# andrewrosemberg/DiffOpt.jl

Hardware: AMD Instinct MI355X
Metric: KKT sensitivity solves/sec (fwd+rev) on batched QPs (higher is better)
Workload: dtype f64; 1 GPU; config 2: dense QP batch, fwd+rev sensitivities; problems_per_gpu=1024, n=200, m_ineq=300, p_eq=0, parallelism=batch-sharded x1

## Files before the change

diffopt.jl_amd/csrc/dopt_internal.h:

```cpp
#pragma once
#include <hip/hip_runtime.h>

#include <cstdint>
#include <functional>
#include <string>
#include <vector>

#include "../../include/diffopt_mi355x.h"

#define DOPT_CHECK_HIP(expr)                                                   \
  do {                                                                         \
    hipError_t _e = (expr);                                                    \
    if (_e != hipSuccess) {                                                    \
      throw dopt::Error(-2, std::string(#expr) + ": " + hipGetErrorString(_e)); \
    }                                                                          \
  } while (0)

namespace dopt {

struct Error {
  int code;
  std::string msg;
  Error(int c, std::string m) : code(c), msg(std::move(m)) {}
};
// ... 5 lines not shown
    if (nbytes <= bytes && p) return;
    if (p) (void)hipFree(p);
    p = nullptr;
    bytes = 0;
    if (nbytes == 0) return;
    DOPT_CHECK_HIP(hipMalloc(&p, nbytes));
    bytes = nbytes;
  }
  void release() {
    if (p) (void)hipFree(p);
    p = nullptr;
    bytes = 0;
  }
  template <class T>
  T* as() const { return static_cast<T*>(p); }
};

enum QPLu { LU_NONE = 0, LU_NOPIV = 1, LU_PIVOT = 2, LU_REJECT = 3, LU_GENERIC = 4, LU_SMALL = 5 };
constexpr int LU_SEL_NOPIV = 1 << LU_NOPIV;
constexpr int LU_SEL_PIVOT = 1 << LU_PIVOT;
constexpr int LU_SEL_ALL = LU_SEL_NOPIV | LU_SEL_PIVOT;
struct QPMeta {
  int32_t nk;
  int32_t nsys;
  int32_t iterative;
  int32_t info;
  int32_t lu;
  int32_t gk_ok;
  int32_t sym;
  int32_t spec_miss;
};

constexpr int ASM_WPP = 16;
constexpr int SM_MAX = 128;
constexpr int SM_BATCH = 8;
constexpr int DENSE_QP_MAX = 8192;
constexpr int BLOCKED_MAX = 4096;
constexpr int PIVOT_MAX = 1536;

enum QPRoute { ROUTE_LSQR = 0, ROUTE_BLOCKED = 2, ROUTE_GENERIC = 3 };
__host__ __device__ inline int qp_route(int iterative, int nsys) {
  if (iterative) return ROUTE_LSQR;
  if (nsys <= BLOCKED_MAX) return ROUTE_BLOCKED;
  return ROUTE_GENERIC;
}

constexpr double NOPIV_LMAX = 10.0;
constexpr double NOPIV_GROWTH = 1e8;

__device__ __forceinline__ double add_mul_rn(double x, double y, double z) {
#pragma clang fp contract(off)
  return x + y * z;
}
__device__ __forceinline__ double sub_rn(double x, double y) {
#pragma clang fp contract(off)
  return x - y;
}

struct PScale {
  const double* kl;
  int n, nk;
  __device__ double operator()(int r) const {
    if (!kl) return 1.0;
    const bool in = r >= n && r < n + nk;
    const double v = kl[in ? r - n : 0];
    return in ? v : 1.0;
// ... 327 lines not shown
```

diffopt.jl_amd/csrc/qp.hip:

```cpp
#include "device_prims.h"
#include "lsqr_core.h"
#include "qp_assemble.h"

namespace dopt {

constexpr int TPB = 256;
constexpr int OUT_LCAP = 4096;
constexpr int NB = 32;

__global__ __launch_bounds__(TPB) void qp_lu_generic_kernel(
    double* __restrict__ K, int32_t* __restrict__ ipiv, QPMeta* __restrict__ meta,
    int nmax, int ld, const int32_t* __restrict__ plist) {
  __shared__ double redv[4];
  __shared__ int redi[4];
  const int b = plist[blockIdx.x], t = threadIdx.x;
  const int lane = t & 63, wv = t >> 6;
  const int N = meta[b].nsys;
  double* Kb = K + (size_t)b * nmax * ld;
  int32_t* piv = ipiv + (size_t)b * nmax;
  int info = 0;
  for (int j = 0; j < N; ++j) {
    double best = -1.0;
    int bi = 0x7fffffff;
    for (int r = j + t; r < N; r += TPB) {
// ... 194 lines not shown
__global__ __launch_bounds__(TPB) void qp_lsqr_kernel(
    const double* __restrict__ K, const QPMeta* __restrict__ meta, int nmax,
    int ld, int trans, const double* __restrict__ rhs, double* __restrict__ xout,
    double* __restrict__ work) {
  __shared__ double red[4];
  const int b = blockIdx.x, t = threadIdx.x;
  if (!meta[b].iterative) return;
  const int N = meta[b].nsys;
  const double* Kb = K + (size_t)b * nmax * ld;
  double* x = work + (size_t)b * 5 * nmax;
  double* u = x + N;
  double* v = u + N;
  double* w = v + N;
  double* tmp = w + N;
  const DenseKKT op{Kb, ld, N, trans};
  LsqrScalars st;
  lsqr_solve<TPB, block_sum>(st, op, rhs + (size_t)b * nmax, 0.0, N, x, u, v, w, tmp, N, red);
  __syncthreads();
  for (int i = t; i < N; i += TPB) xout[(size_t)b * nmax + i] = x[i];
}

__global__ __launch_bounds__(TPB) void qp_rev_rhs_kernel(
    const double* __restrict__ dl_dz, const QPMeta* __restrict__ meta, int n,
    int nmax, double* __restrict__ rhs, double* __restrict__ rhs2) {
  const int b = blockIdx.x, t = threadIdx.x;
  const int N = meta[b].nsys;
  for (int i = t; i < N; i += TPB) {
    const double v = (i < n) ? dl_dz[(size_t)b * n + i] : 0.0;
    rhs[(size_t)b * nmax + i] = v;
    if (rhs2) rhs2[(size_t)b * nmax + i] = v;
  }
}

__global__ __launch_bounds__(TPB) void qp_fwd_rhs_kernel(
    const double* __restrict__ dQ, const double* __restrict__ dq,
    const double* __restrict__ dG, const double* __restrict__ dh,
    const double* __restrict__ dA, const double* __restrict__ db,
    const double* __restrict__ z, const double* __restrict__ lam,
    const double* __restrict__ nu, const int32_t* __restrict__ rpos,
    const QPMeta* __restrict__ meta, int n, int m, int p, int nmax, int zcap,
    double* __restrict__ full, double* __restrict__ rhs, double* __restrict__ rhs2) {
  extern __shared__ __attribute__((aligned(16))) double smem[];
  const int b = blockIdx.x, t = threadIdx.x, lane = t & 63, wv = t >> 6;
  const double* zg = z + (size_t)b * n;
  const double* lb = lam + (size_t)b * m;
  const double* nb = nu + (size_t)b * p;
  const bool staged = n <= zcap;
  if (staged)
    for (int i = t; i < n; i += TPB) smem[i] = zg[i];
  __syncthreads();
  const double* zs = staged ? smem : zg;
  double* r = full + (size_t)b * nmax;
  for (int i = t; i < n; i += TPB) {
    double acc = 0.0;
    if (dQ) {
      const double* Qb = dQ + (size_t)b * n * n;
      for (int j = 0; j < n; ++j) acc = fma(Qb[i + (size_t)j * n], zs[j], acc);
    }
    if (dq) acc += dq[(size_t)b * n + i];
    r[i] = acc;
  }
  __syncthreads();
  if (dG && m > 0) {
    const double* Gb = dG + (size_t)b * m * n;
    for (int i = wv; i < n; i += 4) {
      double acc = 0.0;
      for (int l = lane; l < m; l += 64) acc = fma(Gb[l + (size_t)i * m], lb[l], acc);
      acc = wave_sum(acc);
      if (lane == 0) r[i] += acc;
    }
  }
  __syncthreads();
  if (dA && p > 0) {
    const double* Ab = dA + (size_t)b * p * n;
    for (int i = wv; i < n; i += 4) {
      double acc = 0.0;
      for (int l = lane; l < p; l += 64) acc = fma(Ab[l + (size_t)i * p], nb[l], acc);
      acc = wave_sum(acc);
      if (lane == 0) r[i] += acc;
    }
  }
  for (int l = t; l < m; l += TPB) {
    double gz = 0.0;
    if (dG) {
      const double* Gb = dG + (size_t)b * m * n;
      for (int j = 0; j < n; ++j) gz = fma(Gb[l + (size_t)j * m], zs[j], gz);
    }
    const double hh = dh ? dh[(size_t)b * m + l] : 0.0;
    r[n + l] = lb[l] * gz - lb[l] * hh;
  }
  for (int e = t; e < p; e += TPB) {
    double az = 0.0;
    if (dA) {
      const double* Ab = dA + (size_t)b * p * n;
      for (int j = 0; j < n; ++j) az = fma(Ab[e + (size_t)j * p], zs[j], az);
    }
    r[n + m + e] = az - (db ? db[(size_t)b * p + e] : 0.0);
  }
  __syncthreads();
  const int nk = meta[b].nk;
  double* rb = rhs + (size_t)b * nmax;
  double* rb2 = rhs2 ? rhs2 + (size_t)b * nmax : nullptr;
  for (int i = t; i < n; i += TPB) {
    rb[i] = r[i];
    if (rb2) rb2[i] = r[i];
  }
  for (int l = t; l < m; l += TPB) {
    const int kk = rpos[(size_t)b * m + l];
    if (kk >= 0) {
      rb[n + kk] = r[n + l];
      if (rb2) rb2[n + kk] = r[n + l];
    }
  }
  for (int e = t; e < p; e += TPB) {
    rb[n + nk + e] = r[n + m + e];
    if (rb2) rb2[n + nk + e] = r[n + m + e];
  }
}

#ifndef DOPT_QP_NT
#define DOPT_QP_NT 0
#endif
__global__ __launch_bounds__(TPB) void qp_output_kernel(
    const double* __restrict__ x0, const double* __restrict__ G,
    const double* __restrict__ s, const int32_t* __restrict__ rpos,
    const QPMeta* __restrict__ meta, const double* __restrict__ full, int n,
    int m, int p, int nmax, int zcap, int trans0, double* __restrict__ out0, const double* __restrict__ x1,
    double* __restrict__ out1, int B) {
  extern __shared__ __attribute__((aligned(16))) double smem[];
  __shared__ int nel;
  const bool second = x1 && (int)blockIdx.x >= B;
  const int b = second ? (int)blockIdx.x - B : (int)blockIdx.x, t = threadIdx.x;
  const double* __restrict__ x = second ? x1 : x0;
  double* __restrict__ out = second ? out1 : out0;
  const int trans = second ? 1 : trans0;
  const int nk = meta[b].nk;
  const double* xb = x + (size_t)b * nmax;
  double* ob = out + (size_t)b * (n + m + p);
  const bool staged = n <= zcap;
  const double* xz = staged ? smem : xb;
  int* el = reinterpret_cast<int*>(smem + (staged ? n : 0));
  const bool listed = !trans && m <= OUT_LCAP;
  if (t == 0) nel = 0;
  for (int i = t; i < n; i += TPB) {
    if (staged) smem[i] = xb[i];
    ob[i] = -xb[i];
  }
  for (int e = t; e < p; e += TPB) ob[n + m + e] = -xb[n + nk + e];
  __syncthreads();
  const double* Gb = G + (size_t)b * m * n;
  const double* sb = s + (size_t)b * m;
  auto elim_row = [&](int l) {
    double acc = 0.0;
    int j = 0;
    for (; j + 8 <= n; j += 8) {
      double gv[8];
#pragma unroll
      for (int u = 0; u < 8; ++u)
        gv[u] = DOPT_QP_NT ? __builtin_nontemporal_load(&Gb[l + (size_t)(j + u) * m]) : Gb[l + (size_t)(j + u) * m];
#pragma unroll
      for (int u = 0; u < 8; ++u) acc = fma(gv[u], xz[j + u], acc);
    }
    for (; j < n; ++j) acc = fma(Gb[l + (size_t)j * m], xz[j], acc);
    ob[n + l] = -((0.0 - acc) / sb[l]);
  };
  for (int l = t; l < m; l += TPB) {
    const int kk = rpos[(size_t)b * m + l];
    if (kk >= 0) {
      ob[n + l] = -xb[n + kk];
    } else if (!trans) {
      if (listed) el[atomicAdd(&nel, 1)] = l;
      else elim_row(l);
    } else {
      ob[n + l] = -(full[(size_t)b * nmax + n + l] / sb[l]);
    }
  }
  if (!listed) return;
  __syncthreads();
  for (int e = t; e < nel; e += TPB) elim_row(el[e]);
}

constexpr int OKC = 16;
__global__ __launch_bounds__(TPB) void qp_output_k_kernel(
    const double* __restrict__ x, const double* __restrict__ G, const double* __restrict__ s,
    const int32_t* __restrict__ rpos, const QPMeta* __restrict__ meta, const double* __restrict__ full,
    int B, int k, int n, int m, int p, int nmax, int trans, double* __restrict__ out) {
  extern __shared__ __attribute__((aligned(16))) double smem[];
  const int b = blockIdx.x, t = threadIdx.x;
  const int j0 = blockIdx.y * OKC, kc = min(OKC, k - j0);
  const int nk = meta[b].nk;
  const size_t L = (size_t)n + m + p;
  const bool staged = !trans && n * OKC * 8 <= 48 * 1024;
  for (int c = 0; c < kc; ++c) {
    const double* xb = x + ((size_t)(j0 + c) * B + b) * nmax;
    double* ob = out + ((size_t)(j0 + c) * B + b) * L;
    for (int i = t; i < n; i += TPB) {
      if (staged) smem[i * OKC + c] = xb[i];
      ob[i] = -xb[i];
    }
    for (int e = t; e < p; e += TPB) ob[n + m + e] = -xb[n + nk + e];
  }
  __syncthreads();
  const double* Gb = G + (size_t)b * m * n;
  for (int l = t; l < m; l += TPB) {
    const int kk = rpos[(size_t)b * m + l];
    const double sl = s[(size_t)b * m + l];
    if (kk >= 0 || trans) {
      for (int c = 0; c < kc; ++c) {
        const size_t pj = (size_t)(j0 + c) * B + b;
        const double xl = kk >= 0 ? x[pj * nmax + n + kk] : full[pj * nmax + n + l] / sl;
        out[pj * L + n + l] = -xl;
      }
      continue;
    }
    double acc[OKC];
#pragma unroll
    for (int c = 0; c < OKC; ++c) acc[c] = 0.0;
    for (int j = 0; j < n; ++j) {
      const double gv = Gb[l + (size_t)j * m];
#pragma unroll
      for (int c = 0; c < OKC; ++c) {
        if (c < kc) {
          const double xz = staged ? smem[j * OKC + c] : x[((size_t)(j0 + c) * B + b) * nmax + j];
          acc[c] = fma(gv, xz, acc[c]);
        }
      }
    }
#pragma unroll
    for (int c = 0; c < OKC; ++c)
      if (c < kc) out[((size_t)(j0 + c) * B + b) * L + n + l] = -((0.0 - acc[c]) / sl);
  }
}

__global__ __launch_bounds__(TPB) void qp_reverse_grads_kernel(
    const double* __restrict__ rev, const double* __restrict__ z, const double* __restrict__ lam,
    const double* __restrict__ nu, int B, int n, int m, int p, double* __restrict__ dQ,
    double* __restrict__ dq, double* __restrict__ dG, double* __restrict__ gc,
    double* __restrict__ dA, double* __restrict__ ac) {
  const int L = n + m + p;
  const long long nn = (long long)n * n, mn = (long long)m * n, pn = (long long)p * n;
  const long long per = nn + mn + pn + n + m + p;
  for (int b = blockIdx.y; b < B; b += gridDim.y) {
    const double* rb = rev + (size_t)b * L;
    const double* zb = z + (size_t)b * n;
    for (long long e = (long long)blockIdx.x * TPB + threadIdx.x; e < per;
         e += (long long)gridDim.x * TPB) {
      if (e < nn) {
        if (!dQ) continue;
        const int i = (int)(e % n), j = (int)(e / n);
        dQ[(size_t)b * nn + e] = 0.5 * (rb[i] * zb[j] + zb[i] * rb[j]);
      } else if (e < nn + mn) {
        if (!dG) continue;
        const long long f = e - nn;
        const int i = (int)(f % m), j = (int)(f / m);
        const double li = lam[(size_t)b * m + i];
        dG[(size_t)b * mn + f] = li * rb[n + i] * zb[j] + li * rb[j];
// ... 96 lines not shown
  P.p = h.p;
  return P;
}

static int32_t* rpos_of(Handle& h) { return h.kidx.as<int32_t>() + (size_t)h.batch * h.m; }

template <class F>
static void prep_assemble(Handle& h, const int32_t* plist, int count, bool full, F&& after_prep) {
  if (count == 0) return;
  const QPIn P = qp_inputs(h);
  if (!full && h.n > 0) {
    ensure_aux(h);
    h.qsy.ensure((size_t)h.batch * (sizeof(double) + sizeof(int32_t)));
    DOPT_CHECK_HIP(hipEventRecord(h.ev_fork, h.stream));
    DOPT_CHECK_HIP(hipStreamWaitEvent(h.aux, h.ev_fork, 0));
    DOPT_CHECK_HIP(hipMemsetAsync(h.qsy.p, 0, h.qsy.bytes, h.aux));
    hipLaunchKernelGGL(qp_qsym_kernel, dim3((unsigned)qsym_pairs(h.n), (unsigned)count), dim3(256), 0, h.aux, P,
                       qsy_max(h), qsy_flag(h), plist);
    check_launch();
    DOPT_CHECK_HIP(hipEventRecord(h.ev_qsym, h.aux));
    h.qsym_pending = true;
  }
  const dim3 pg(count), pb(prep_threads(h.m));
  if (prep_rows_per_thread(h.m) == 2)
    hipLaunchKernelGGL(qp_prep_kernel<2>, pg, pb, prep_lds(h.n), h.stream, P, h.s.as<double>(),
                       h.kidx.as<int32_t>(), rpos_of(h), h.kls.as<double>(), h.gk.as<double>(), h.batch, h.meta.as<QPMeta>(),
                       plist, h.kamax.as<double>(), h.sym_mode);
  else
    hipLaunchKernelGGL(qp_prep_kernel<1>, pg, pb, prep_lds(h.n), h.stream, P, h.s.as<double>(),
                       h.kidx.as<int32_t>(), rpos_of(h), h.kls.as<double>(), h.gk.as<double>(), h.batch, h.meta.as<QPMeta>(),
                       plist, h.kamax.as<double>(), h.sym_mode);
  check_launch();
  after_prep();
  hipLaunchKernelGGL(qp_asm_tile_kernel, dim3((unsigned)count * ASM_WPP), dim3(512), 0, h.stream, P,
                     h.kidx.as<int32_t>(), h.kls.as<double>(), h.gk.as<double>(), h.batch, h.meta.as<QPMeta>(),
                     h.K.as<double>(), h.ld,
                     h.nmax, plist, full ? 1 : 0, h.kamax.as<double>());
  check_launch();
}
static void prep_assemble(Handle& h, const int32_t* plist, int count) { prep_assemble(h, plist, count, true, [] {}); }

static void meta_copy(Handle& h) {
  if (!h.meta_host) {
    DOPT_CHECK_HIP(hipHostMalloc((void**)&h.meta_host, std::max<size_t>(h.batch, 1) * sizeof(QPMeta)));
    DOPT_CHECK_HIP(hipEventCreateWithFlags(&h.meta_ev, hipEventDisableTiming));
  }
  DOPT_CHECK_HIP(hipMemcpyAsync(h.meta_host, h.meta.p, h.batch * sizeof(QPMeta), hipMemcpyDeviceToHost,
                                h.stream));
  DOPT_CHECK_HIP(hipEventRecord(h.meta_ev, h.stream));
}

static void meta_copy_side(Handle& h) {
  ensure_aux(h);
  if (!h.meta_host) {
    DOPT_CHECK_HIP(hipHostMalloc((void**)&h.meta_host, std::max<size_t>(h.batch, 1) * sizeof(QPMeta)));
    DOPT_CHECK_HIP(hipEventCreateWithFlags(&h.meta_ev, hipEventDisableTiming));
  }
  DOPT_CHECK_HIP(hipEventRecord(h.meta_fork, h.stream));
  DOPT_CHECK_HIP(hipStreamWaitEvent(h.crit, h.meta_fork, 0));
  DOPT_CHECK_HIP(hipMemcpyAsync(h.meta_host, h.meta.p, h.batch * sizeof(QPMeta), hipMemcpyDeviceToHost, h.crit));
  DOPT_CHECK_HIP(hipEventRecord(h.meta_ev, h.crit));
}

static void meta_sizes(Handle& h) {
  DOPT_CHECK_HIP(hipEventSynchronize(h.meta_ev));
  int npmax = 0;
  h.has_generic = h.has_lsqr = false;
  for (int64_t b = 0; b < h.batch; ++b) {
    const QPMeta& mm = h.meta_host[b];
    const int r = qp_route(mm.iterative, mm.nsys);
// ... 143 lines not shown
  check_launch();
}

static double* rhs_of(Handle& h, int trans) {
  return h.rhs.as<double>() + (size_t)(trans ? 2 : 0) * h.batch * h.nmax;
}
static double* full_of(Handle& h) { return h.rhs.as<double>() + (size_t)h.batch * h.nmax; }
static double* x_of(Handle& h, int trans) {
  return h.x.as<double>() + (size_t)(trans ? 1 : 0) * h.batch * h.nmax;
}

static void finish_into(Handle& h, int trans, double* rhs, double* x, const double* full, double* out,
                        const double* pair_x = nullptr, double* pair_out = nullptr, bool solves_only = false) {
  const int B = (int)h.batch, n = h.n, m = h.m, p = h.p;
  const int nmax = h.nmax, ld = h.ld;
  QPMeta* meta = h.meta.as<QPMeta>();
  if (h.n_generic > 0) {
    PhaseTimer pt(h, DOPT_PHASE_QP_SOLVE);
    if ((size_t)nmax * sizeof(double) > 64 * 1024) throw Error(-1, "generic solve: system too large");
    hipLaunchKernelGGL(qp_solve_kernel, dim3(B), dim3(TPB), (size_t)nmax * sizeof(double), h.stream,
                       h.K.as<double>(), h.ipiv.as<int32_t>(), meta, nmax, ld, trans, rhs, x);
    check_launch();
  }
  if (h.has_lsqr) {
    PhaseTimer pt(h, DOPT_PHASE_QP_LSQR);
    h.lsqr_ws.ensure((size_t)B * 5 * nmax * sizeof(double));
    hipLaunchKernelGGL(qp_lsqr_kernel, dim3(B), dim3(TPB), 0, h.stream, h.K.as<double>(), meta, nmax, ld,
                       trans, rhs, x, h.lsqr_ws.as<double>());
    check_launch();
  }
  if (solves_only) return;
  static const double dummy = 0.0;
  PhaseTimer pt(h, DOPT_PHASE_QP_OUTPUT);
  const size_t olds = (n <= ZCAP ? (size_t)n * sizeof(double) : 0) +
                      (!trans && m <= OUT_LCAP ? (size_t)m * sizeof(int) : 0);
  if (pair_x) {
    hipLaunchKernelGGL(qp_output_kernel, dim3(2 * B), dim3(TPB), olds, h.stream, x, m ? h.G : &dummy,
                       h.s.as<double>(), rpos_of(h), meta, full, n, m, p, nmax, ZCAP, 0, out, pair_x, pair_out, B);
  } else {
    hipLaunchKernelGGL(qp_output_kernel, dim3(B), dim3(TPB), olds, h.stream, x, m ? h.G : &dummy,
                       h.s.as<double>(), rpos_of(h), meta, full, n, m, p, nmax, ZCAP, trans, out,
                       (const double*)nullptr, (double*)nullptr, B);
  }
  check_launch();
}
static void finish(Handle& h, int trans, double* out) {
  finish_into(h, trans, rhs_of(h, trans), x_of(h, trans), full_of(h), out);
}
static void finish_pair(Handle& h, double* out_rev, double* out_fwd) {
  finish_into(h, 1, rhs_of(h, 1), x_of(h, 1), full_of(h), nullptr, nullptr, nullptr, true);
  finish_into(h, 0, rhs_of(h, 0), x_of(h, 0), full_of(h), out_rev, x_of(h, 1), out_fwd);
}

static void rev_rhs(Handle& h, const double* dl_dz, double* copy = nullptr) {
  PhaseTimer pt(h, DOPT_PHASE_QP_RHS);
  hipLaunchKernelGGL(qp_rev_rhs_kernel, dim3(h.batch), dim3(TPB), 0, h.stream, dl_dz, h.meta.as<QPMeta>(),
                     h.n, h.nmax, rhs_of(h, 0), copy);
  check_launch();
}

static void fwd_rhs_into(Handle& h, const FwdTangents& T, double* full, double* rhs, double* copy = nullptr) {
  const int B = (int)h.batch, n = h.n, m = h.m, p = h.p;
  static const double dummy = 0.0;
  hipLaunchKernelGGL(qp_fwd_rhs_kernel, dim3(B), dim3(TPB), (size_t)std::min(n, ZCAP) * sizeof(double),
                     h.stream, T.dQ, T.dq, T.dG, T.dh, T.dA, T.db, h.z, m ? h.lam : &dummy,
                     p ? h.nu : &dummy, rpos_of(h), h.meta.as<QPMeta>(), n, m, p, h.nmax, ZCAP, full, rhs, copy);
  check_launch();
}
static void fwd_rhs(Handle& h, const FwdTangents& T, double* copy = nullptr) {
  PhaseTimer pt(h, DOPT_PHASE_QP_RHS);
  fwd_rhs_into(h, T, full_of(h), rhs_of(h, 1), copy);
}

static FwdTangents tangents(Handle& h, const double* dQ, const double* dq, const double* dG,
                            const double* dh, const double* dA, const double* db) {
  FwdTangents T;
  T.dQ = dQ;
  T.dq = dq;
  T.dG = h.m ? dG : nullptr;
  T.dh = h.m ? dh : nullptr;
  T.dA = h.p ? dA : nullptr;
  T.db = h.p ? db : nullptr;
  return T;
}

void qp_reverse(Handle& h, const double* dl_dz, double* out) {
  if (!h.factored) qp_factor(h);
  rev_rhs(h, dl_dz);
  {
    PhaseTimer pt(h, DOPT_PHASE_QP_SOLVE);
    qp_blocked_solve(h, dinv_of(h), 0, rhs_of(h, 0), x_of(h, 0), LU_SEL_ALL);
  }
  finish(h, 0, out);
}

void qp_forward(Handle& h, const double* dQ, const double* dq, const double* dG,
                const double* dh, const double* dA, const double* db, double* out) {
  if (!h.factored) qp_factor(h);
  fwd_rhs(h, tangents(h, dQ, dq, dG, dh, dA, db));
// ... 4 lines not shown
  finish(h, 1, out);
}

static void solve_k(Handle& h, int trans, int k, double* rk, double* xk, double* fk, double* out) {
  const size_t blk = (size_t)h.batch * h.nmax;
  const int B = (int)h.batch, n = h.n, m = h.m, p = h.p, nmax = h.nmax;
  {
    PhaseTimer pt(h, DOPT_PHASE_QP_SOLVE);
    qp_blocked_solve_multi(h, dinv_of(h), trans, k, rk, xk, LU_SEL_ALL);
  }
  QPMeta* meta = h.meta.as<QPMeta>();
  for (int j = 0; j < k; ++j) {
    double* rhs = rk + j * blk;
    double* x = xk + j * blk;
    if (h.n_generic > 0) {
      PhaseTimer pt(h, DOPT_PHASE_QP_SOLVE);
      if ((size_t)nmax * sizeof(double) > 64 * 1024) throw Error(-1, "generic solve: system too large");
      hipLaunchKernelGGL(qp_solve_kernel, dim3(B), dim3(TPB), (size_t)nmax * sizeof(double), h.stream,
                         h.K.as<double>(), h.ipiv.as<int32_t>(), meta, nmax, h.ld, trans, rhs, x);
      check_launch();
    }
    if (h.has_lsqr) {
      PhaseTimer pt(h, DOPT_PHASE_QP_LSQR);
      h.lsqr_ws.ensure((size_t)B * 5 * nmax * sizeof(double));
      hipLaunchKernelGGL(qp_lsqr_kernel, dim3(B), dim3(TPB), 0, h.stream, h.K.as<double>(), meta, nmax, h.ld,
                         trans, rhs, x, h.lsqr_ws.as<double>());
      check_launch();
    }
  }
  static const double dummy = 0.0;
  PhaseTimer pt(h, DOPT_PHASE_QP_OUTPUT);
  const int nck = (k + OKC - 1) / OKC;
  const size_t lds = (!trans && (size_t)n * OKC * 8 <= 48 * 1024) ? (size_t)n * OKC * 8 : 0;
  hipLaunchKernelGGL(qp_output_k_kernel, dim3(B, nck), dim3(TPB), lds, h.stream, xk, m ? h.G : &dummy,
                     h.s.as<double>(), rpos_of(h), meta, fk ? fk : xk, B, k, n, m, p, nmax, trans, out);
  check_launch();
}

void qp_reverse_k(Handle& h, int k, const double* dl_dz, double* out) {
  if (k <= 0) throw Error(-1, "dopt_qp_reverse_k: k must be positive");
  if (k == 1) return qp_reverse(h, dl_dz, out);
  if (!h.factored) qp_factor(h);
  const size_t blk = (size_t)h.batch * h.nmax;
  h.krhs.ensure((size_t)k * blk * sizeof(double));
  h.kx.ensure((size_t)k * blk * sizeof(double));
  double* rk = h.krhs.as<double>();
  double* xk = h.kx.as<double>();
  {
    PhaseTimer pt(h, DOPT_PHASE_QP_RHS);
    for (int j = 0; j < k; ++j) {
      hipLaunchKernelGGL(qp_rev_rhs_kernel, dim3(h.batch), dim3(TPB), 0, h.stream, dl_dz + (size_t)j * h.batch * h.n,
                         h.meta.as<QPMeta>(), h.n, h.nmax, rk + j * blk, nullptr);
      check_launch();
    }
  }
  solve_k(h, 0, k, rk, xk, nullptr, out);
}

void qp_forward_k(Handle& h, int k, const double* dQ, const double* dq, const double* dG, const double* dh,
                  const double* dA, const double* db, double* out) {
  if (k <= 0) throw Error(-1, "dopt_qp_forward_k: k must be positive");
  if (k == 1) return qp_forward(h, dQ, dq, dG, dh, dA, db, out);
  if (!h.factored) qp_factor(h);
  const size_t B = h.batch, n = h.n, m = h.m, p = h.p;
  const size_t blk = B * h.nmax;
  h.krhs.ensure((size_t)k * blk * sizeof(double));
  h.kx.ensure((size_t)k * blk * sizeof(double));
// ... 2 lines not shown
  double* xk = h.kx.as<double>();
  double* fk = h.kfull.as<double>();
  {
    PhaseTimer pt(h, DOPT_PHASE_QP_RHS);
    for (int j = 0; j < k; ++j) {
      auto at = [&](const double* a, size_t len) { return a ? a + (size_t)j * B * len : nullptr; };
      const FwdTangents T = tangents(h, at(dQ, n * n), at(dq, n), at(dG, m * n), at(dh, m), at(dA, p * n),
                                     at(db, p));
      fwd_rhs_into(h, T, fk + j * blk, rk + j * blk);
    }
  }
  solve_k(h, 1, k, rk, xk, fk, out);
}

void qp_reverse_grads(Handle& h, const double* rev, double* dQ, double* dq, double* dG, double* gc,
                      double* dA, double* ac) {
  if (!h.set) throw Error(-1, "dopt_qp_reverse_grads: dopt_qp_set has not been called");
  static const double dummy = 0.0;
  const long long per = (long long)h.n * h.n + (long long)(h.m + h.p) * h.n + h.n + h.m + h.p;
  const int gx = (int)std::max<long long>(1, std::min<long long>((per + TPB - 1) / TPB, 64));
  const int gy = (int)std::min<int64_t>(h.batch, 65535);
  hipLaunchKernelGGL(qp_reverse_grads_kernel, dim3(gx, gy), dim3(TPB), 0, h.stream, rev, h.z,
                     h.m ? h.lam : &dummy, h.p ? h.nu : &dummy, (int)h.batch, h.n, h.m, h.p, dQ, dq,
                     h.m ? dG : nullptr, h.m ? gc : nullptr, h.p ? dA : nullptr, h.p ? ac : nullptr);
  check_launch();
}

void qp_forward_reverse(Handle& h, const double* dl_dz, const double* dQ,
                        const double* dq, const double* dG, const double* dh,
                        const double* dA, const double* db, double* out_rev,
                        double* out_fwd) {
  if (!h.set) throw Error(-1, "dopt_qp_forward_reverse: dopt_qp_set has not been called");
  const FwdTangents T = tangents(h, dQ, dq, dG, dh, dA, db);
  {
    PhaseTimer pt(h, DOPT_PHASE_QP_ASSEMBLE);
    prep_assemble(h, nullptr, (int)h.batch, h.lu_mode == 0, [&] { meta_copy_side(h); });
  }
  double *w0 = nullptr, *w1 = nullptr;
  if (h.lu_mode == 1) {
    const size_t len = (size_t)h.batch * h.nmax;
    h.fwdw.ensure(2 * len * sizeof(double));
    w0 = h.fwdw.as<double>();
    w1 = w0 + len;
  }
  rev_rhs(h, dl_dz, w0);
  fwd_rhs(h, T, w1);
  meta_sizes(h);
  if (!h.blocked_npmax) w0 = w1 = nullptr;
  auto solve2 = [&](int sel, const double* sw0, const double* sw1) {
    PhaseTimer pt(h, DOPT_PHASE_QP_SOLVE);
    qp_blocked_solve2(h, dinv_of(h), rhs_of(h, 0), rhs_of(h, 1), x_of(h, 0), x_of(h, 1), sel, sw0, sw1);
  };
  const bool spec_out = h.lu_mode == 1 && !h.has_generic && !h.has_lsqr;
  h.n_generic = 0;
  factor_blocked(
      h,
      [&] {
        solve2(h.lu_mode == 1 ? LU_SEL_NOPIV : LU_SEL_ALL, w0, w1);
        if (spec_out) finish_pair(h, out_rev, out_fwd);
      },
      w0, w1, qp_reasm(h));
  if (h.n_pivot > 0) solve2(LU_SEL_PIVOT, nullptr, nullptr);
  if (!spec_out || h.n_pivot > 0 || h.n_generic > 0) finish_pair(h, out_rev, out_fwd);
  h.factored = true;
  h.info_clear = h.lu_mode == 1 && h.n_pivot == 0 && h.n_generic == 0;
}

}
```

diffopt.jl_amd/csrc/qp_assemble.h:

```cpp
#pragma once

#include "dopt_internal.h"

namespace dopt {

template <int RPT>
__global__ void qp_prep_kernel(QPIn, double*, int32_t*, int32_t*, double*, double*, int64_t, QPMeta*,
                               const int32_t*, double*, int);
__global__ void qp_asm_tile_kernel(QPIn, const int32_t*, const double*, const double*, int64_t, QPMeta*, double*,
                                   int, int, const int32_t*, int, double*);
__global__ void qp_qsym_kernel(QPIn, double*, int32_t*, const int32_t*);
int qsym_pairs(int n);
int prep_rows_per_thread(int m);
int prep_threads(int m);
size_t prep_lds(int n);

}
```

diffopt.jl_amd/csrc/qp_assemble.hip:

```cpp
#include "qp_assemble.h"

namespace dopt {

constexpr int PREP_U = 16;
constexpr int PREP_U2 = 8;
constexpr int PREP_MAXT = 256;
constexpr int ZLDS_MAX = 8192;
constexpr int BUF_FLAGS = 0x00020000;

typedef double dv2 __attribute__((ext_vector_type(2)));
typedef unsigned int u32v2 __attribute__((ext_vector_type(2)));
typedef unsigned int u32v4 __attribute__((ext_vector_type(4)));
#ifndef DOPT_QP_NT
#define DOPT_QP_NT 0
#endif
__device__ __forceinline__ dv2 bload2(__amdgpu_buffer_rsrc_t r, unsigned off) {
  return __builtin_bit_cast(dv2, __builtin_amdgcn_raw_buffer_load_b128(r, off, 0, DOPT_QP_NT ? 2 : 0));
}
__device__ __forceinline__ void bstore1(__amdgpu_buffer_rsrc_t r, unsigned off, double x) {
  __builtin_amdgcn_raw_buffer_store_b64(__builtin_bit_cast(u32v2, x), r, off, 0, 0);
}

template <int RPT>
__global__ __launch_bounds__(PREP_MAXT, 3) void qp_prep_kernel(QPIn P, double* __restrict__ s_out,
                                                            int32_t* __restrict__ kidx, int32_t* __restrict__ rpos,
                                                            double* __restrict__ kls, double* __restrict__ gk,
                                                            int64_t B, QPMeta* __restrict__ meta,
                                                            const int32_t* __restrict__ plist,
                                                            double* __restrict__ kamax, int sym_mode) {
  extern __shared__ __attribute__((aligned(16))) double zdyn[];
  __shared__ int cnt[PREP_MAXT / 64 + 1], scnt[PREP_MAXT / 64 + 1];
  __shared__ int extra, asym;
  __shared__ double kred[PREP_MAXT / 64];
  double kmx = 0.0;
  const int t = threadIdx.x, lane = t & 63, wv = t >> 6;
  const int T = (int)blockDim.x, NW = T >> 6;
  const int b = plist ? plist[blockIdx.x] : (int)blockIdx.x;
  const int n = P.n, m = P.m, p = P.p;
  const double* Qb = P.Q + (size_t)b * n * n;
  int iterative = 1;
  {
    const size_t nn = (size_t)n * n;
    for (size_t i0 = 0; i0 < nn; i0 += (size_t)8 * T) {
      int nz = 0;
      double q[8];
#pragma unroll
      for (int u = 0; u < 8; ++u) {
        const size_t i = i0 + (size_t)u * T + t;
        q[u] = Qb[i < nn ? i : 0];
      }
#pragma unroll
      for (int u = 0; u < 8; ++u) nz |= (q[u] != 0.0);
      if (__syncthreads_or(nz)) { iterative = 0; break; }
    }
  }
  const bool zl = n <= ZLDS_MAX;
  if (zl)
    for (int j = t; j < n; j += T) zdyn[j] = P.z[(size_t)b * n + j];
  const double* zs = zl ? zdyn : P.z + (size_t)b * n;
  if (t == 0) {
    cnt[NW] = 0;
    scnt[NW] = 0;
    extra = 0;
    asym = 0;
  }
  __syncthreads();
  const double* Gb = P.G + (size_t)b * m * n;
  double* gkb = gk + (size_t)b * n * m;
  const double* lb = P.lam + (size_t)b * m;
  const double* hb = P.h + (size_t)b * m;
  const unsigned long long lt = (1ull << lane) - 1ull;
  for (int i0 = 0; i0 < m; i0 += RPT * T) {
    const int i = i0 + RPT * t;
    bool valid[RPT];
    double acc[RPT], li[RPT];
    int spec[RPT];
#pragma unroll
    for (int q = 0; q < RPT; ++q) {
      valid[q] = i + q < m;
      acc[q] = 0.0;
      li[q] = valid[q] ? lb[i + q] : 0.0;
      spec[q] = valid[q] && (iterative || li[q] != 0.0);
    }
    int sci[RPT];
    double gm[RPT];
#pragma unroll
    for (int q = 0; q < RPT; ++q) gm[q] = 0.0;
    {
      int sbelow = 0, scount = 0;
#pragma unroll
      for (int q = 0; q < RPT; ++q) {
        const unsigned long long ball = __ballot(spec[q]);
        sbelow += __popcll(ball & lt);
        scount += __popcll(ball);
      }
      if (lane == 0) scnt[wv] = scount;
      __syncthreads();
      int soff = scnt[NW];
      for (int w = 0; w < wv; ++w) soff += scnt[w];
#pragma unroll
      for (int q = 0; q < RPT; ++q) sci[q] = soff + sbelow + (q ? spec[0] : 0);
    }
    {
      const double* gp = Gb + (valid[RPT - 1] ? i : 0);
      double* gw0 = gkb + sci[0];
      int j = 0;
      if constexpr (RPT == 2) {
        const unsigned bytes = (unsigned)((size_t)n * m * sizeof(double));
        const __amdgpu_buffer_rsrc_t gr = __builtin_amdgcn_make_buffer_rsrc(const_cast<double*>(Gb), 0, bytes, BUF_FLAGS);
        const __amdgpu_buffer_rsrc_t wr = __builtin_amdgcn_make_buffer_rsrc(gkb, 0, bytes, BUF_FLAGS);
        const unsigned mb = (unsigned)m * 8u, lo = (unsigned)(valid[1] ? i : 0) * 8u;
        const unsigned so0 = spec[0] ? (unsigned)sci[0] * 8u : 0x80000000u;
        const unsigned so1 = spec[1] ? (unsigned)sci[1] * 8u : 0x80000000u;
        dv2 cur[PREP_U2], nxt[PREP_U2];
        if (PREP_U2 <= n) {
#pragma unroll
          for (int u = 0; u < PREP_U2; ++u) cur[u] = bload2(gr, lo + (unsigned)u * mb);
        }
        for (; j + PREP_U2 <= n; j += PREP_U2) {
          const bool more = j + 2 * PREP_U2 <= n;
          if (more) {
#pragma unroll
            for (int u = 0; u < PREP_U2; ++u) nxt[u] = bload2(gr, lo + (unsigned)(j + PREP_U2 + u) * mb);
          }
#pragma unroll
          for (int u = 0; u < PREP_U2; ++u) {
            acc[0] = add_mul_rn(acc[0], cur[u].x, zs[j + u]);
            acc[1] = add_mul_rn(acc[1], cur[u].y, zs[j + u]);
            gm[0] = fmax(gm[0], fabs(cur[u].x));
            gm[1] = fmax(gm[1], fabs(cur[u].y));
            bstore1(wr, so0 + (unsigned)(j + u) * mb, cur[u].x);
            bstore1(wr, so1 + (unsigned)(j + u) * mb, cur[u].y);
          }
          if (more) {
#pragma unroll
            for (int u = 0; u < PREP_U2; ++u) cur[u] = nxt[u];
          }
        }
        for (; j < n; ++j) {
          const dv2 g2 = bload2(gr, lo + (unsigned)j * mb);
          acc[0] = add_mul_rn(acc[0], g2.x, zs[j]);
          acc[1] = add_mul_rn(acc[1], g2.y, zs[j]);
          gm[0] = fmax(gm[0], fabs(g2.x));
          gm[1] = fmax(gm[1], fabs(g2.y));
          bstore1(wr, so0 + (unsigned)j * mb, g2.x);
          bstore1(wr, so1 + (unsigned)j * mb, g2.y);
        }
      } else {
        for (; j + PREP_U <= n; j += PREP_U) {
          double gv[PREP_U];
#pragma unroll
          for (int u = 0; u < PREP_U; ++u) gv[u] = gp[(size_t)(j + u) * m];
#pragma unroll
          for (int u = 0; u < PREP_U; ++u) {
            acc[0] = add_mul_rn(acc[0], gv[u], zs[j + u]);
            gm[0] = fmax(gm[0], fabs(gv[u]));
            if (spec[0]) gw0[(size_t)(j + u) * m] = gv[u];
          }
        }
        for (; j < n; ++j) {
          const double g = gp[(size_t)j * m];
          acc[0] = add_mul_rn(acc[0], g, zs[j]);
          gm[0] = fmax(gm[0], fabs(g));
          if (spec[0]) gw0[(size_t)j * m] = g;
        }
      }
    }
    int keep[RPT];
    double si[RPT];
#pragma unroll
    for (int q = 0; q < RPT; ++q) {
      keep[q] = 0;
      si[q] = 0.0;
      if (valid[q]) {
        si[q] = sub_rn(acc[q], hb[i + q]);
        s_out[(size_t)b * m + i + q] = si[q];
        keep[q] = iterative ? 1 : !(li[q] == 0.0 && si[q] != 0.0);
        if (keep[q] && !spec[q]) atomicAdd(&extra, 1);
        if (keep[q] && !(fabs(li[q]) > 0.0 && fabs(li[q]) <= 1.7976931348623157e308)) asym = 1;
        if (keep[q]) kmx = fmax(kmx, fmax(fmax(gm[q], gm[q] * fabs(li[q])), fabs(si[q])));
      }
    }
    int prefix[RPT], wcount = 0, below = 0;
#pragma unroll
    for (int q = 0; q < RPT; ++q) {
      const unsigned long long ball = __ballot(keep[q]);
      below += __popcll(ball & lt);
      wcount += __popcll(ball);
    }
#pragma unroll
    for (int q = 0; q < RPT; ++q) prefix[q] = below + (q ? keep[0] : 0);
    if (lane == 0) cnt[wv] = wcount;
    __syncthreads();
    int off = cnt[NW];
    for (int w = 0; w < wv; ++w) off += cnt[w];
// ... 17 lines not shown
        ssum += scnt[w];
      }
      cnt[NW] += sum;
      scnt[NW] += ssum;
    }
    __syncthreads();
  }
  for (int o = 32; o > 0; o >>= 1) kmx = fmax(kmx, __shfl_xor(kmx, o));
  if (lane == 0) kred[wv] = kmx;
  __syncthreads();
  if (t == 0) {
    for (int w = 1; w < NW; ++w) kmx = fmax(kmx, kred[w]);
    const int nk = cnt[NW];
    meta[b].nk = nk;
    meta[b].nsys = n + nk + p;
    meta[b].iterative = iterative;
    meta[b].info = 0;
    meta[b].lu = LU_NONE;
    meta[b].gk_ok = extra == 0;
    meta[b].sym = sym_mode && !asym && qp_route(iterative, n + nk + p) == ROUTE_BLOCKED;
    kamax[b] = kmx;
  }
}
template __global__ void qp_prep_kernel<1>(QPIn, double*, int32_t*, int32_t*, double*, double*, int64_t, QPMeta*,
                                           const int32_t*, double*, int);
template __global__ void qp_prep_kernel<2>(QPIn, double*, int32_t*, int32_t*, double*, double*, int64_t, QPMeta*,
                                           const int32_t*, double*, int);

int prep_rows_per_thread(int m) { return (m % 2 == 0) ? 2 : 1; }
int prep_threads(int m) {
  const int rows = (m + prep_rows_per_thread(m) - 1) / prep_rows_per_thread(m);
  return std::min(PREP_MAXT, std::max(64, (rows + 63) & ~63));
}
size_t prep_lds(int n) { return n <= ZLDS_MAX ? (size_t)std::max(n, 1) * sizeof(double) : 0; }

constexpr int AT = 64, ATLD = AT + 2, ATH = 512;
constexpr int AK1 = AT * AT / ATH;

__global__ __launch_bounds__(ATH) void qp_asm_tile_kernel(QPIn P, const int32_t* __restrict__ kidx,
                                                          const double* __restrict__ kls,
                                                          const double* __restrict__ gk, int64_t B,
                                                          QPMeta* __restrict__ meta, double* __restrict__ Kper,
                                                          int ld, int nmax, const int32_t* __restrict__ plist,
                                                          int full, double* __restrict__ kamax) {
  __shared__ __attribute__((aligned(16))) double Ts[2][AT * ATLD];
  __shared__ int kid_s[2][AT];
  __shared__ double lam_s[2][AT], s_s[2][AT];
  const int t = threadIdx.x;
  const int slot = (int)blockIdx.x / ASM_WPP, g = (int)blockIdx.x % ASM_WPP;
  const int b = plist ? plist[slot] : slot;
  const int n = P.n, m = P.m, p = P.p;
  const int nk = meta[b].nk;
  const bool gk_ok = meta[b].gk_ok != 0;
  if (!full && meta[b].sym != 0) return;
  const int N = n + nk + p, Np = (N + 31) & ~31, TT = (Np + AT - 1) / AT;
  const int npairs = TT * (TT + 1) / 2;
  if (g >= npairs) return;
  double* K = Kper + (size_t)b * nmax * ld;
  const double* Qb = P.Q + (size_t)b * n * n;
  const double* Gb = P.G + (size_t)b * m * n;
  const double* Ab = P.A + (size_t)b * p * n;
  const int32_t* kb = kidx + (size_t)b * m;
  const double* lkb = kls + (size_t)b * m;
  const double* skb = kls + ((size_t)B + b) * m;
  const double* gkb = gk + (size_t)b * n * m;
  auto grow = [&](int rng, int e, int ci) { return gk_ok ? gkb + ci : Gb + kid_s[rng][e]; };
  const int tr = t & 63, tc = t >> 6;
  const int scol = t & 63, srow = t >> 6;

  auto tile_load = [&](int r0, int c0, int rng_r, int rng_c, double* Tl) {
    const double* vbase = nullptr;
    size_t vstride = 0;
    if (c0 < n && r0 + AT <= Np) {
      if (r0 + AT <= n && (n & 1) == 0) { vbase = Qb + r0; vstride = n; }
      else if (gk_ok && r0 >= n && r0 + AT <= n + nk && ((r0 - n) & 1) == 0 && (m & 1) == 0) {
        vbase = gkb + (r0 - n); vstride = m;
      }
    }
    if (vbase) {
      const int rp = t & 31, cg = t >> 5;
      dv2 w[AT / 16];
#pragma unroll
// ... 42 lines not shown
      } else if (c < N) {
        base = Ab + (c - n - nk); rs = p; dval = 0.0;
      } else {
        cok = false;
      }
      double v[AK1];
#pragma unroll
      for (int k = 0; k < AK1; ++k) {
        const int r = r0 + srow + 8 * k;
        v[k] = base[(size_t)((cok && r < n) ? r : 0) * rs];
      }
#pragma unroll
      for (int k = 0; k < AK1; ++k) {
        const int r = r0 + srow + 8 * k;
        Tl[(srow + 8 * k) * ATLD + scol] = r < n ? (cok ? (gcol ? v[k] * li : v[k]) : 0.0) : (r == c ? dval : 0.0);
      }
    }
  };
  double vmax = 0.0;
  auto tile_store = [&](int r0, int c0, const double* Tl) {
    const int cp = 2 * (t & 31), rw = t >> 5;
    if (c0 + cp >= Np) return;
#pragma unroll
    for (int k = 0; k < AT / 16; ++k) {
      const int rr = rw + 16 * k, r = r0 + rr;
      if (r < Np) {
        const double2 v = *reinterpret_cast<const double2*>(Tl + rr * ATLD + cp);
        *reinterpret_cast<double2*>(K + (size_t)r * ld + c0 + cp) = v;
        vmax = fmax(vmax, fmax(fabs(v.x), fabs(v.y)));
      }
    }
  };

  for (int q = g; q < npairs; q += ASM_WPP) {
    int R = 0, rem = q;
    while (rem >= TT - R) { rem -= TT - R; ++R; }
    const int C = R + rem;
    if (t < 2 * AT) {
      const int which = t >> 6, e = t & 63;
      const int ci = (which ? C : R) * AT + e - n;
      const bool ok = ci >= 0 && ci < nk;
      kid_s[which][e] = ok ? kb[ci] : 0;
      lam_s[which][e] = ok ? lkb[ci] : 0.0;
      s_s[which][e] = ok ? skb[ci] : 0.0;
    }
    __syncthreads();
    tile_load(R * AT, C * AT, 0, 1, Ts[0]);
    if (R != C) tile_load(C * AT, R * AT, 1, 0, Ts[1]);
    __syncthreads();
    tile_store(R * AT, C * AT, Ts[0]);
    if (R != C) tile_store(C * AT, R * AT, Ts[1]);
    __syncthreads();
  }
  for (int o = 32; o > 0; o >>= 1) vmax = fmax(vmax, __shfl_xor(vmax, o));
  if ((t & 63) == 0)
    atomicMax(reinterpret_cast<unsigned long long*>(kamax) + b, (unsigned long long)__double_as_longlong(vmax));
}

constexpr int QS = 64, QSLD = QS + 1, QST = 256;

__global__ __launch_bounds__(QST) void qp_qsym_kernel(QPIn P, double* __restrict__ qmax, int32_t* __restrict__ qflag,
                                                      const int32_t* __restrict__ plist) {
  __shared__ double T[QS * QSLD];
  const int b = plist ? plist[blockIdx.y] : (int)blockIdx.y;
  const int n = P.n, t = threadIdx.x;
  const int TQ = (n + QS - 1) / QS;
  int R = 0, rem = (int)blockIdx.x;
// ... 49 lines not shown
```

Measured before the change: 890,400 solves/s.

## Overlap RHS building with assembly, template staging, cap assembly workgroups, double-buffer prep loads

The forward and reverse right-hand-side kernels now launch inside the assembly side-callback, so they can overlap with the prepare/assemble phase instead of running after it. The asm tile kernel takes a runtime workgroups-per-problem value, capped at a total workgroup budget when assembly is not full, which reduces oversubscription at large batch. The output and fwd_rhs kernels are templated on whether z/x is staged in LDS, removing runtime branches. The prepare kernel always stages z in LDS and uses an explicit two-buffer software pipeline for G loads. These are several unrelated tweaks, and the side-callback ordering relies on the rhs kernels not depending on assembly results.

```diff
diff --git a/diffopt.jl_amd/csrc/dopt_internal.h b/diffopt.jl_amd/csrc/dopt_internal.h
--- a/diffopt.jl_amd/csrc/dopt_internal.h
+++ b/diffopt.jl_amd/csrc/dopt_internal.h
@@ -61,6 +61,7 @@
 };
 
 constexpr int ASM_WPP = 16;
+constexpr int ASM_SPEC_WGS = 4096;
 constexpr int SM_MAX = 128;
 constexpr int SM_BATCH = 8;
 constexpr int DENSE_QP_MAX = 8192;
diff --git a/diffopt.jl_amd/csrc/qp.hip b/diffopt.jl_amd/csrc/qp.hip
--- a/diffopt.jl_amd/csrc/qp.hip
+++ b/diffopt.jl_amd/csrc/qp.hip
@@ -250,30 +250,33 @@
   }
 }
 
+template <bool STAGED>
 __global__ __launch_bounds__(TPB) void qp_fwd_rhs_kernel(
     const double* __restrict__ dQ, const double* __restrict__ dq,
     const double* __restrict__ dG, const double* __restrict__ dh,
     const double* __restrict__ dA, const double* __restrict__ db,
     const double* __restrict__ z, const double* __restrict__ lam,
     const double* __restrict__ nu, const int32_t* __restrict__ rpos,
-    const QPMeta* __restrict__ meta, int n, int m, int p, int nmax, int zcap,
+    const QPMeta* __restrict__ meta, int n, int m, int p, int nmax,
     double* __restrict__ full, double* __restrict__ rhs, double* __restrict__ rhs2) {
   extern __shared__ __attribute__((aligned(16))) double smem[];
   const int b = blockIdx.x, t = threadIdx.x, lane = t & 63, wv = t >> 6;
   const double* zg = z + (size_t)b * n;
   const double* lb = lam + (size_t)b * m;
   const double* nb = nu + (size_t)b * p;
-  const bool staged = n <= zcap;
-  if (staged)
+  if constexpr (STAGED)
     for (int i = t; i < n; i += TPB) smem[i] = zg[i];
   __syncthreads();
-  const double* zs = staged ? smem : zg;
+  auto zs = [&](int j) {
+    if constexpr (STAGED) return smem[j];
+    else return zg[j];
+  };
   double* r = full + (size_t)b * nmax;
   for (int i = t; i < n; i += TPB) {
     double acc = 0.0;
     if (dQ) {
       const double* Qb = dQ + (size_t)b * n * n;
-      for (int j = 0; j < n; ++j) acc = fma(Qb[i + (size_t)j * n], zs[j], acc);
+      for (int j = 0; j < n; ++j) acc = fma(Qb[i + (size_t)j * n], zs(j), acc);
     }
     if (dq) acc += dq[(size_t)b * n + i];
     r[i] = acc;
@@ -302,7 +305,7 @@
     double gz = 0.0;
     if (dG) {
       const double* Gb = dG + (size_t)b * m * n;
-      for (int j = 0; j < n; ++j) gz = fma(Gb[l + (size_t)j * m], zs[j], gz);
+      for (int j = 0; j < n; ++j) gz = fma(Gb[l + (size_t)j * m], zs(j), gz);
     }
     const double hh = dh ? dh[(size_t)b * m + l] : 0.0;
     r[n + l] = lb[l] * gz - lb[l] * hh;
@@ -311,7 +314,7 @@
     double az = 0.0;
     if (dA) {
       const double* Ab = dA + (size_t)b * p * n;
-      for (int j = 0; j < n; ++j) az = fma(Ab[e + (size_t)j * p], zs[j], az);
+      for (int j = 0; j < n; ++j) az = fma(Ab[e + (size_t)j * p], zs(j), az);
     }
     r[n + m + e] = az - (db ? db[(size_t)b * p + e] : 0.0);
   }
@@ -339,11 +342,12 @@
 #ifndef DOPT_QP_NT
 #define DOPT_QP_NT 0
 #endif
+template <bool STAGED>
 __global__ __launch_bounds__(TPB) void qp_output_kernel(
     const double* __restrict__ x0, const double* __restrict__ G,
     const double* __restrict__ s, const int32_t* __restrict__ rpos,
     const QPMeta* __restrict__ meta, const double* __restrict__ full, int n,
-    int m, int p, int nmax, int zcap, int trans0, double* __restrict__ out0, const double* __restrict__ x1,
+    int m, int p, int nmax, int trans0, double* __restrict__ out0, const double* __restrict__ x1,
     double* __restrict__ out1, int B) {
   extern __shared__ __attribute__((aligned(16))) double smem[];
   __shared__ int nel;
@@ -355,13 +359,15 @@
   const int nk = meta[b].nk;
   const double* xb = x + (size_t)b * nmax;
   double* ob = out + (size_t)b * (n + m + p);
-  const bool staged = n <= zcap;
-  const double* xz = staged ? smem : xb;
-  int* el = reinterpret_cast<int*>(smem + (staged ? n : 0));
+  auto xz = [&](int j) {
+    if constexpr (STAGED) return smem[j];
+    else return xb[j];
+  };
+  int* el = reinterpret_cast<int*>(smem + (STAGED ? n : 0));
   const bool listed = !trans && m <= OUT_LCAP;
   if (t == 0) nel = 0;
   for (int i = t; i < n; i += TPB) {
-    if (staged) smem[i] = xb[i];
+    if constexpr (STAGED) smem[i] = xb[i];
     ob[i] = -xb[i];
   }
   for (int e = t; e < p; e += TPB) ob[n + m + e] = -xb[n + nk + e];
@@ -377,9 +383,9 @@
       for (int u = 0; u < 8; ++u)
         gv[u] = DOPT_QP_NT ? __builtin_nontemporal_load(&Gb[l + (size_t)(j + u) * m]) : Gb[l + (size_t)(j + u) * m];
 #pragma unroll
-      for (int u = 0; u < 8; ++u) acc = fma(gv[u], xz[j + u], acc);
-    }
-    for (; j < n; ++j) acc = fma(Gb[l + (size_t)j * m], xz[j], acc);
+      for (int u = 0; u < 8; ++u) acc = fma(gv[u], xz(j + u), acc);
+    }
+    for (; j < n; ++j) acc = fma(Gb[l + (size_t)j * m], xz(j), acc);
     ob[n + l] = -((0.0 - acc) / sb[l]);
   };
   for (int l = t; l < m; l += TPB) {
@@ -399,6 +405,7 @@
 }
 
 constexpr int OKC = 16;
+template <bool STAGED>
 __global__ __launch_bounds__(TPB) void qp_output_k_kernel(
     const double* __restrict__ x, const double* __restrict__ G, const double* __restrict__ s,
     const int32_t* __restrict__ rpos, const QPMeta* __restrict__ meta, const double* __restrict__ full,
@@ -408,12 +415,11 @@
   const int j0 = blockIdx.y * OKC, kc = min(OKC, k - j0);
   const int nk = meta[b].nk;
   const size_t L = (size_t)n + m + p;
-  const bool staged = !trans && n * OKC * 8 <= 48 * 1024;
   for (int c = 0; c < kc; ++c) {
     const double* xb = x + ((size_t)(j0 + c) * B + b) * nmax;
     double* ob = out + ((size_t)(j0 + c) * B + b) * L;
     for (int i = t; i < n; i += TPB) {
-      if (staged) smem[i * OKC + c] = xb[i];
+      if constexpr (STAGED) smem[i * OKC + c] = xb[i];
       ob[i] = -xb[i];
     }
     for (int e = t; e < p; e += TPB) ob[n + m + e] = -xb[n + nk + e];
@@ -439,7 +445,9 @@
 #pragma unroll
       for (int c = 0; c < OKC; ++c) {
         if (c < kc) {
-          const double xz = staged ? smem[j * OKC + c] : x[((size_t)(j0 + c) * B + b) * nmax + j];
+          double xz;
+          if constexpr (STAGED) xz = smem[j * OKC + c];
+          else xz = x[((size_t)(j0 + c) * B + b) * nmax + j];
           acc[c] = fma(gv, xz, acc[c]);
         }
       }
@@ -602,10 +610,11 @@
                        plist, h.kamax.as<double>(), h.sym_mode);
   check_launch();
   after_prep();
-  hipLaunchKernelGGL(qp_asm_tile_kernel, dim3((unsigned)count * ASM_WPP), dim3(512), 0, h.stream, P,
+  const int wpp = full ? ASM_WPP : std::max(1, std::min(ASM_WPP, ASM_SPEC_WGS / count));
+  hipLaunchKernelGGL(qp_asm_tile_kernel, dim3((unsigned)count * wpp), dim3(512), 0, h.stream, P,
                      h.kidx.as<int32_t>(), h.kls.as<double>(), h.gk.as<double>(), h.batch, h.meta.as<QPMeta>(),
                      h.K.as<double>(), h.ld,
-                     h.nmax, plist, full ? 1 : 0, h.kamax.as<double>());
+                     h.nmax, plist, full ? 1 : 0, h.kamax.as<double>(), wpp);
   check_launch();
 }
 static void prep_assemble(Handle& h, const int32_t* plist, int count) { prep_assemble(h, plist, count, true, [] {}); }
@@ -815,14 +824,16 @@
   if (solves_only) return;
   static const double dummy = 0.0;
   PhaseTimer pt(h, DOPT_PHASE_QP_OUTPUT);
-  const size_t olds = (n <= ZCAP ? (size_t)n * sizeof(double) : 0) +
+  const bool staged = n <= ZCAP;
+  const size_t olds = (staged ? (size_t)n * sizeof(double) : 0) +
                       (!trans && m <= OUT_LCAP ? (size_t)m * sizeof(int) : 0);
+  const auto kern = staged ? qp_output_kernel<true> : qp_output_kernel<false>;
   if (pair_x) {
-    hipLaunchKernelGGL(qp_output_kernel, dim3(2 * B), dim3(TPB), olds, h.stream, x, m ? h.G : &dummy,
-                       h.s.as<double>(), rpos_of(h), meta, full, n, m, p, nmax, ZCAP, 0, out, pair_x, pair_out, B);
+    hipLaunchKernelGGL(kern, dim3(2 * B), dim3(TPB), olds, h.stream, x, m ? h.G : &dummy,
+                       h.s.as<double>(), rpos_of(h), meta, full, n, m, p, nmax, 0, out, pair_x, pair_out, B);
   } else {
-    hipLaunchKernelGGL(qp_output_kernel, dim3(B), dim3(TPB), olds, h.stream, x, m ? h.G : &dummy,
-                       h.s.as<double>(), rpos_of(h), meta, full, n, m, p, nmax, ZCAP, trans, out,
+    hipLaunchKernelGGL(kern, dim3(B), dim3(TPB), olds, h.stream, x, m ? h.G : &dummy,
+                       h.s.as<double>(), rpos_of(h), meta, full, n, m, p, nmax, trans, out,
                        (const double*)nullptr, (double*)nullptr, B);
   }
   check_launch();
@@ -845,9 +856,11 @@
 static void fwd_rhs_into(Handle& h, const FwdTangents& T, double* full, double* rhs, double* copy = nullptr) {
   const int B = (int)h.batch, n = h.n, m = h.m, p = h.p;
   static const double dummy = 0.0;
-  hipLaunchKernelGGL(qp_fwd_rhs_kernel, dim3(B), dim3(TPB), (size_t)std::min(n, ZCAP) * sizeof(double),
+  const bool staged = n <= ZCAP;
+  hipLaunchKernelGGL(staged ? qp_fwd_rhs_kernel<true> : qp_fwd_rhs_kernel<false>, dim3(B), dim3(TPB),
+                     staged ? (size_t)n * sizeof(double) : 0,
                      h.stream, T.dQ, T.dq, T.dG, T.dh, T.dA, T.db, h.z, m ? h.lam : &dummy,
-                     p ? h.nu : &dummy, rpos_of(h), h.meta.as<QPMeta>(), n, m, p, h.nmax, ZCAP, full, rhs, copy);
+                     p ? h.nu : &dummy, rpos_of(h), h.meta.as<QPMeta>(), n, m, p, h.nmax, full, rhs, copy);
   check_launch();
 }
 static void fwd_rhs(Handle& h, const FwdTangents& T, double* copy = nullptr) {
@@ -918,7 +931,7 @@
   PhaseTimer pt(h, DOPT_PHASE_QP_OUTPUT);
   const int nck = (k + OKC - 1) / OKC;
   const size_t lds = (!trans && (size_t)n * OKC * 8 <= 48 * 1024) ? (size_t)n * OKC * 8 : 0;
-  hipLaunchKernelGGL(qp_output_k_kernel, dim3(B, nck), dim3(TPB), lds, h.stream, xk, m ? h.G : &dummy,
+  hipLaunchKernelGGL(lds ? qp_output_k_kernel<true> : qp_output_k_kernel<false>, dim3(B, nck), dim3(TPB), lds, h.stream, xk, m ? h.G : &dummy,
                      h.s.as<double>(), rpos_of(h), meta, fk ? fk : xk, B, k, n, m, p, nmax, trans, out);
   check_launch();
 }
@@ -987,10 +1000,6 @@
                         double* out_fwd) {
   if (!h.set) throw Error(-1, "dopt_qp_forward_reverse: dopt_qp_set has not been called");
   const FwdTangents T = tangents(h, dQ, dq, dG, dh, dA, db);
-  {
-    PhaseTimer pt(h, DOPT_PHASE_QP_ASSEMBLE);
-    prep_assemble(h, nullptr, (int)h.batch, h.lu_mode == 0, [&] { meta_copy_side(h); });
-  }
   double *w0 = nullptr, *w1 = nullptr;
   if (h.lu_mode == 1) {
     const size_t len = (size_t)h.batch * h.nmax;
@@ -998,8 +1007,17 @@
     w0 = h.fwdw.as<double>();
     w1 = w0 + len;
   }
-  rev_rhs(h, dl_dz, w0);
-  fwd_rhs(h, T, w1);
+  auto rhs_pair = [&] {
+    rev_rhs(h, dl_dz, w0);
+    fwd_rhs(h, T, w1);
+  };
+  {
+    PhaseTimer pt(h, DOPT_PHASE_QP_ASSEMBLE);
+    prep_assemble(h, nullptr, (int)h.batch, h.lu_mode == 0, [&] {
+      meta_copy_side(h);
+      rhs_pair();
+    });
+  }
   meta_sizes(h);
   if (!h.blocked_npmax) w0 = w1 = nullptr;
   auto solve2 = [&](int sel, const double* sw0, const double* sw1) {
diff --git a/diffopt.jl_amd/csrc/qp_assemble.h b/diffopt.jl_amd/csrc/qp_assemble.h
--- a/diffopt.jl_amd/csrc/qp_assemble.h
+++ b/diffopt.jl_amd/csrc/qp_assemble.h
@@ -8,7 +8,7 @@
 __global__ void qp_prep_kernel(QPIn, double*, int32_t*, int32_t*, double*, double*, int64_t, QPMeta*,
                                const int32_t*, double*, int);
 __global__ void qp_asm_tile_kernel(QPIn, const int32_t*, const double*, const double*, int64_t, QPMeta*, double*,
-                                   int, int, const int32_t*, int, double*);
+                                   int, int, const int32_t*, int, double*, int);
 __global__ void qp_qsym_kernel(QPIn, double*, int32_t*, const int32_t*);
 int qsym_pairs(int n);
 int prep_rows_per_thread(int m);
diff --git a/diffopt.jl_amd/csrc/qp_assemble.hip b/diffopt.jl_amd/csrc/qp_assemble.hip
--- a/diffopt.jl_amd/csrc/qp_assemble.hip
+++ b/diffopt.jl_amd/csrc/qp_assemble.hip
@@ -54,10 +54,7 @@
       if (__syncthreads_or(nz)) { iterative = 0; break; }
     }
   }
-  const bool zl = n <= ZLDS_MAX;
-  if (zl)
-    for (int j = t; j < n; j += T) zdyn[j] = P.z[(size_t)b * n + j];
-  const double* zs = zl ? zdyn : P.z + (size_t)b * n;
+  for (int j = t; j < n; j += T) zdyn[j] = P.z[(size_t)b * n + j];
   if (t == 0) {
     cnt[NW] = 0;
     scnt[NW] = 0;
@@ -112,35 +109,50 @@
         const unsigned mb = (unsigned)m * 8u, lo = (unsigned)(valid[1] ? i : 0) * 8u;
         const unsigned so0 = spec[0] ? (unsigned)sci[0] * 8u : 0x80000000u;
         const unsigned so1 = spec[1] ? (unsigned)sci[1] * 8u : 0x80000000u;
-        dv2 cur[PREP_U2], nxt[PREP_U2];
-        if (PREP_U2 <= n) {
-#pragma unroll
-          for (int u = 0; u < PREP_U2; ++u) cur[u] = bload2(gr, lo + (unsigned)u * mb);
-        }
-        for (; j + PREP_U2 <= n; j += PREP_U2) {
-          const bool more = j + 2 * PREP_U2 <= n;
-          if (more) {
-#pragma unroll
-            for (int u = 0; u < PREP_U2; ++u) nxt[u] = bload2(gr, lo + (unsigned)(j + PREP_U2 + u) * mb);
+        dv2 ga[PREP_U2], gb[PREP_U2];
+        auto issue = [&](dv2(&g)[PREP_U2], int c) {
+#pragma unroll
+          for (int u = 0; u < PREP_U2; ++u) g[u] = bload2(gr, lo + (unsigned)(c * PREP_U2 + u) * mb);
+        };
+        auto take = [&](const dv2(&g)[PREP_U2], int c) {
+          const int jc = c * PREP_U2;
+#pragma unroll
+          for (int u = 0; u < PREP_U2; ++u) {
+            acc[0] = add_mul_rn(acc[0], g[u].x, zdyn[jc + u]);
+            acc[1] = add_mul_rn(acc[1], g[u].y, zdyn[jc + u]);
+            gm[0] = fmax(gm[0], fabs(g[u].x));
+            gm[1] = fmax(gm[1], fabs(g[u].y));
+            bstore1(wr, so0 + (unsigned)(jc + u) * mb, g[u].x);
+            bstore1(wr, so1 + (unsigned)(jc + u) * mb, g[u].y);
           }
-#pragma unroll
-          for (int u = 0; u < PREP_U2; ++u) {
-            acc[0] = add_mul_rn(acc[0], cur[u].x, zs[j + u]);
-            acc[1] = add_mul_rn(acc[1], cur[u].y, zs[j + u]);
-            gm[0] = fmax(gm[0], fabs(cur[u].x));
-            gm[1] = fmax(gm[1], fabs(cur[u].y));
-            bstore1(wr, so0 + (unsigned)(j + u) * mb, cur[u].x);
-            bstore1(wr, so1 + (unsigned)(j + u) * mb, cur[u].y);
+        };
+        const int C = n / PREP_U2;
+        if (C == 1) {
+          issue(ga, 0);
+          take(ga, 0);
+        } else if (C >= 2) {
+          issue(ga, 0);
+          issue(gb, 1);
+          take(ga, 0);
+          int c = 1;
+          for (; c + 2 < C; c += 2) {
+            issue(ga, c + 1);
+            take(gb, c);
+            issue(gb, c + 2);
+            take(ga, c + 1);
           }
-          if (more) {
-#pragma unroll
-            for (int u = 0; u < PREP_U2; ++u) cur[u] = nxt[u];
+          if (c + 1 < C) {
+            issue(ga, c + 1);
+            take(gb, c);
+            take(ga, c + 1);
+          } else {
+            take(gb, c);
           }
         }
-        for (; j < n; ++j) {
+        for (j = C * PREP_U2; j < n; ++j) {
           const dv2 g2 = bload2(gr, lo + (unsigned)j * mb);
-          acc[0] = add_mul_rn(acc[0], g2.x, zs[j]);
-          acc[1] = add_mul_rn(acc[1], g2.y, zs[j]);
+          acc[0] = add_mul_rn(acc[0], g2.x, zdyn[j]);
+          acc[1] = add_mul_rn(acc[1], g2.y, zdyn[j]);
           gm[0] = fmax(gm[0], fabs(g2.x));
           gm[1] = fmax(gm[1], fabs(g2.y));
           bstore1(wr, so0 + (unsigned)j * mb, g2.x);
@@ -153,14 +165,14 @@
           for (int u = 0; u < PREP_U; ++u) gv[u] = gp[(size_t)(j + u) * m];
 #pragma unroll
           for (int u = 0; u < PREP_U; ++u) {
-            acc[0] = add_mul_rn(acc[0], gv[u], zs[j + u]);
+            acc[0] = add_mul_rn(acc[0], gv[u], zdyn[j + u]);
             gm[0] = fmax(gm[0], fabs(gv[u]));
             if (spec[0]) gw0[(size_t)(j + u) * m] = gv[u];
           }
         }
         for (; j < n; ++j) {
           const double g = gp[(size_t)j * m];
-          acc[0] = add_mul_rn(acc[0], g, zs[j]);
+          acc[0] = add_mul_rn(acc[0], g, zdyn[j]);
           gm[0] = fmax(gm[0], fabs(g));
           if (spec[0]) gw0[(size_t)j * m] = g;
         }
@@ -244,7 +256,11 @@
   const int rows = (m + prep_rows_per_thread(m) - 1) / prep_rows_per_thread(m);
   return std::min(PREP_MAXT, std::max(64, (rows + 63) & ~63));
 }
-size_t prep_lds(int n) { return n <= ZLDS_MAX ? (size_t)std::max(n, 1) * sizeof(double) : 0; }
+static_assert(ZLDS_MAX >= DENSE_QP_MAX, "the prepare kernel stages all of z in LDS");
+size_t prep_lds(int n) {
+  if (n > ZLDS_MAX) throw Error(-1, "qp prepare: n above the dense route's cap (z is staged in LDS)");
+  return (size_t)std::max(n, 1) * sizeof(double);
+}
 
 constexpr int AT = 64, ATLD = AT + 2, ATH = 512;
 constexpr int AK1 = AT * AT / ATH;
@@ -254,12 +270,12 @@
                                                           const double* __restrict__ gk, int64_t B,
                                                           QPMeta* __restrict__ meta, double* __restrict__ Kper,
                                                           int ld, int nmax, const int32_t* __restrict__ plist,
-                                                          int full, double* __restrict__ kamax) {
+                                                          int full, double* __restrict__ kamax, int wpp) {
   __shared__ __attribute__((aligned(16))) double Ts[2][AT * ATLD];
   __shared__ int kid_s[2][AT];
   __shared__ double lam_s[2][AT], s_s[2][AT];
   const int t = threadIdx.x;
-  const int slot = (int)blockIdx.x / ASM_WPP, g = (int)blockIdx.x % ASM_WPP;
+  const int slot = (int)blockIdx.x / wpp, g = (int)blockIdx.x % wpp;
   const int b = plist ? plist[slot] : slot;
   const int n = P.n, m = P.m, p = P.p;
   const int nk = meta[b].nk;
@@ -368,7 +384,7 @@
     }
   };
 
-  for (int q = g; q < npairs; q += ASM_WPP) {
+  for (int q = g; q < npairs; q += wpp) {
     int R = 0, rem = q;
     while (rem >= TT - R) { rem -= TT - R; ++R; }
     const int C = R + rem;
```

Result: no change. 891,000 solves/s, median of 4 (+0.1%).
